# MarvelMathesh/sincformer-metacog-speech-enhancement

Measured on AMD Instinct MI355X. Metric: audio frames/sec/GPU (16 kHz, 512-frame utts) + mask RMSE vs CPU ref, higher is better.
Workload: dtype fp16 MFMA operands (PerceptionAgent, fusion, Conformer GEMMs, heads) + bf16 attention core, fp32 accumulate (ops.POLICIES['mixed']); 1 GPU; B256 x 512-frame utterances (L40880, T512) forward; batch_per_gpu=256, samples=40880, frames_per_utt=512, launch=eager launches, streams=2, precision_policy=mixed

## Files before the change

sincformer_metacog_speech_enhancement_amd/csrc/sinc_fir16.hip:

```cpp
#include "sfm_common.h"

#define FIR_C 64
#define FIR_KP 272
#define FIR_WROW 280
#define FIR_WAVES 8
#define FIR_SUB (FIR_WAVES * 256)
#define FIR_NSUB 4
#define FIR_XPT ((FIR_SUB + FIR_KP + FIR_WAVES * 64 - 1) / (FIR_WAVES * 64))
#define FIR_SPAN (FIR_SUB + FIR_KP)

template <class T>
__global__ __launch_bounds__(256) void sinc_fir16_prep_kernel(const float* __restrict__ filt, u16* __restrict__ wsh, int K) {
  const int o = blockIdx.x, c = blockIdx.y;
  for (int kp = threadIdx.x; kp < FIR_KP; kp += 256) {
    const int k = kp - o;
    const float h = (k >= 0 && k < K) ? filt[c * K + k] * 4096.0f : 0.f;
    const u16 hi = T::from_f32(h);
    const u16 lo = T::from_f32(h - T::to_f32(hi));
    wsh[(((long long)o * 2 + 0) * FIR_C + c) * FIR_KP + kp] = hi;
    wsh[(((long long)o * 2 + 1) * FIR_C + c) * FIR_KP + kp] = lo;
  }
}

template <class T, int PASSES>
__global__ __launch_bounds__(FIR_WAVES * 64) void sinc_fir16_kernel(const float* __restrict__ sig, const u16* __restrict__ wsh,
                                                         void* __restrict__ out, float* __restrict__ gn_partial,
                                                         int L, int pad, int out_f32, int tiles_per_batch) {
  extern __shared__ __attribute__((aligned(16))) unsigned char dsm[];
  u16* Wh = reinterpret_cast<u16*>(dsm);
  u16* Wl = Wh + FIR_C * FIR_WROW;
  u16* Xh = Wl + FIR_C * FIR_WROW;
  u16* Xl = Xh + FIR_SPAN;
  float* img = reinterpret_cast<float*>(Xl + FIR_SPAN);

  const int tid = threadIdx.x, lane = tid & 63, wave = tid >> 6;
  const int l31 = lane & 31, hl = lane >> 5;
  const int o = blockIdx.x, b = blockIdx.z;
  const int c0 = blockIdx.y * (FIR_NSUB * FIR_SUB);
  const float* xb = sig + (long long)b * L;

  {
    const u16* src = wsh + (long long)o * 2 * FIR_C * FIR_KP;
    for (int e = tid; e < 2 * FIR_C * (FIR_KP / 8); e += FIR_WAVES * 64) {
      const int part = e / (FIR_C * (FIR_KP / 8));
      const int rem = e - part * (FIR_C * (FIR_KP / 8));
      const int c = rem / (FIR_KP / 8), k8 = (rem - c * (FIR_KP / 8)) * 8;
      const u32x4 v = *reinterpret_cast<const u32x4*>(src + ((long long)part * FIR_C + c) * FIR_KP + k8);
      *reinterpret_cast<u32x4*>((part ? Wl : Wh) + c * FIR_WROW + k8) = v;
    }
  }

  constexpr int NT = FIR_WAVES * 64;
  float xr[FIR_XPT];
  auto load_span = [&](int m0) {
#pragma unroll
    for (int q = 0; q < FIR_XPT; ++q) {
      const int i = tid + q * NT;
      const int sidx = m0 + i - pad;
      xr[q] = (i < FIR_SPAN && sidx >= 0 && sidx < L) ? xb[sidx] : 0.f;
    }
  };
  load_span(c0);
  for (int sub = 0; sub < FIR_NSUB; ++sub) {
    const int m0 = c0 + sub * FIR_SUB;
    if (m0 >= L) break;
    __syncthreads();
#pragma unroll
    for (int q = 0; q < FIR_XPT; ++q) {
      const int i = tid + q * NT;
      if (i < FIR_SPAN) {
        const u16 hi = T::from_f32(xr[q]);
        Xh[i] = hi;
        Xl[i] = T::from_f32(xr[q] - T::to_f32(hi));
      }
    }
    __syncthreads();
    if (sub + 1 < FIR_NSUB && m0 + FIR_SUB < L) load_span(m0 + FIR_SUB);

    f32x16 acc[2];
#pragma unroll
    for (int j = 0; j < 2; ++j)
#pragma unroll
      for (int r = 0; r < 16; ++r) acc[j][r] = 0.f;
    const int xoff = wave * 256 + 8 * l31 + 8 * hl;
#pragma unroll
    for (int k0 = 0; k0 < FIR_KP; k0 += 16) {
      const u32x4 ah = *reinterpret_cast<const u32x4*>(Xh + xoff + k0);
      const u32x4 al = *reinterpret_cast<const u32x4*>(Xl + xoff + k0);
#pragma unroll
      for (int j = 0; j < 2; ++j) {
        const int wo = (j * 32 + l31) * FIR_WROW + k0 + 8 * hl;
        const u32x4 bh = *reinterpret_cast<const u32x4*>(Wh + wo);
        const u32x4 bl = *reinterpret_cast<const u32x4*>(Wl + wo);
        acc[j] = T::mfma(ah, bh, acc[j]);
        if (PASSES == 3) {
          acc[j] = T::mfma(ah, bl, acc[j]);
          acc[j] = T::mfma(al, bh, acc[j]);
        }
      }
    }

    float* im = img + wave * (32 * 68);
#pragma unroll
    for (int j = 0; j < 2; ++j)
#pragma unroll
      for (int r = 0; r < 16; ++r) im[mfma_row(r, lane) * 68 + j * 32 + l31] = acc[j][r] * (1.0f / 4096.0f);
    __builtin_amdgcn_s_waitcnt(0xC07F);
    __builtin_amdgcn_wave_barrier();
    const int c8 = (lane & 7) * 8, rsub = lane >> 3;
    float gsum = 0.f, gsq = 0.f;
#pragma unroll
    for (int r0 = 0; r0 < 32; r0 += 8) {
      const int row = r0 + rsub;
      const int m = m0 + wave * 256 + o + 8 * row;
      const f32x4 x0 = *reinterpret_cast<const f32x4*>(&im[row * 68 + c8]);
      const f32x4 x1 = *reinterpret_cast<const f32x4*>(&im[row * 68 + c8 + 4]);
      if (m < L) {
        const float v[8] = {x0[0], x0[1], x0[2], x0[3], x1[0], x1[1], x1[2], x1[3]};
#pragma unroll
        for (int e = 0; e < 8; ++e) { gsum += v[e]; gsq += v[e] * v[e]; }
        const long long off = ((long long)b * L + m) * FIR_C + c8;
        if (out_f32) {
          float* op = reinterpret_cast<float*>(out) + off;
          *reinterpret_cast<f32x4*>(op) = x0;
          *reinterpret_cast<f32x4*>(op + 4) = x1;
        } else {
          u32x4 pk;
#pragma unroll
          for (int e = 0; e < 4; ++e) pk[e] = pack2<T>(v[2 * e], v[2 * e + 1]);
          *reinterpret_cast<u32x4*>(reinterpret_cast<u16*>(out) + off) = pk;
        }
      }
    }
    if (gn_partial) {
      for (int s = 8; s < 64; s <<= 1) {
        gsum += __shfl_xor(gsum, s, 64);
        gsq += __shfl_xor(gsq, s, 64);
      }
      if (lane < 8) {
        const long long tile = ((long long)blockIdx.y * FIR_NSUB + sub) * (8 * FIR_WAVES) + o * FIR_WAVES + wave;
        const long long slot = (((long long)b * tiles_per_batch + tile) * 8 + lane) * 2;
        gn_partial[slot] = gsum;
        gn_partial[slot + 1] = gsq;
      }
    }
  }
}

extern "C" int sfm_sinc_fir16_tiles(int L) {
  const int chunk = FIR_NSUB * FIR_SUB;
  const int nchunks = (L + chunk - 1) / chunk;
  return nchunks * FIR_NSUB * 8 * FIR_WAVES;
}

template <class T, int PASSES>
static int sinc_fir16_go(const float* wave, const float* filt, void* wsh, void* out, float* gn_partial, int L, int K, int out_f32,
                         dim3 grid, int lds, int tpb, hipStream_t st) {
  SFM_LAUNCH((sinc_fir16_prep_kernel<T>), dim3(8, FIR_C), dim3(256), 0, st, filt, (u16*)wsh, K);
  SFM_LAUNCH_LDS((sinc_fir16_kernel<T, PASSES>), grid, dim3(FIR_WAVES * 64), lds, st, wave, (const u16*)wsh, out, gn_partial, L,
                 K / 2, out_f32, tpb);
  return SFM_OK;
}

extern "C" int sfm_sinc_fir16_ex(const float* wave, const float* filt, void* wsh, void* out, float* gn_partial, int B, int L, int C,
                                 int K, int out_f32, int dtype, int passes, void* stream) {
  if (!wave || !filt || !wsh || !out) return SFM_ERR_ARG;
  if (C != FIR_C || K < 1 || K + 7 > FIR_KP || (K & 1) == 0 || B <= 0 || L <= 0 || (passes != 0 && passes != 1 && passes != 3))
    return SFM_ERR_SHAPE;
  hipStream_t st = (hipStream_t)stream;
  const int chunk = FIR_NSUB * FIR_SUB;
  const int nchunks = (L + chunk - 1) / chunk;
  const int lds = (2 * FIR_C * FIR_WROW + 2 * FIR_SPAN) * 2 + FIR_WAVES * 32 * 68 * 4;
  const int tpb = nchunks * FIR_NSUB * 8 * FIR_WAVES;
  dim3 grid(8, nchunks, B);
  if (passes == 0) passes = (dtype == SFM_DT_F16 && out_f32 == 0) ? 1 : 3;
  if (dtype == SFM_DT_F16)
    return passes == 1 ? sinc_fir16_go<F16, 1>(wave, filt, wsh, out, gn_partial, L, K, out_f32, grid, lds, tpb, st)
                       : sinc_fir16_go<F16, 3>(wave, filt, wsh, out, gn_partial, L, K, out_f32, grid, lds, tpb, st);
  return passes == 1 ? sinc_fir16_go<BF16, 1>(wave, filt, wsh, out, gn_partial, L, K, out_f32, grid, lds, tpb, st)
                     : sinc_fir16_go<BF16, 3>(wave, filt, wsh, out, gn_partial, L, K, out_f32, grid, lds, tpb, st);
}

extern "C" int sfm_sinc_fir16(const float* wave, const float* filt, void* wsh, void* out, float* gn_partial, int B,
                              int L, int C, int K, int out_f32, int dtype, void* stream) {
  return sfm_sinc_fir16_ex(wave, filt, wsh, out, gn_partial, B, L, C, K, out_f32, dtype, 0, stream);
}
```

sincformer_metacog_speech_enhancement_amd/ops.py:

```python
import ctypes
import math
import numpy as np
import torch

from . import lib as _lib

EPI_NONE, EPI_SWISH, EPI_GELU, EPI_RESID, EPI_GLU, EPI_SIGMOID, EPI_TANH_SCALE, EPI_SIGMA, EPI_CPEA = range(9)

_DT_ID = {torch.bfloat16: 0, torch.float16: 1}
import os as _os
TRAIN_DTYPE = torch.float16
_state = {"dtype": TRAIN_DTYPE}

_SWITCHES = {
    "gemm_variant": ["SFM_GEMM_VARIANT", 0, 0],
    "attention_variant": [None, 0, 0],
    "lin256": ["SFM_LIN256", True, True],
    "headpool": ["SFM_HEADPOOL", True, True],
    "lstm_w16": ["SFM_LSTM_W16", True, True],
    "deterministic": ["SFM_DETERMINISTIC", True, True],
    "wgrad_stream": ["SFM_WGRAD_STREAM", True, True],
    "fuse_ffn_swish": ["SFM_FUSE_FFN_SWISH", True, True],
    "fuse_next_drop": ["SFM_FUSE_NEXT_DROP", True, True],
    "steal_grads": ["SFM_STEAL_GRADS", False, False],
# ... 528 lines not shown
        else:
            v = 2 if T >= 1024 else 1
    return {1: "attn_fwd_hd64_kernel", 2: "attn_fwd_hd64x2_kernel", 3: "attn_fwd_hd64r_kernel", 4: "attn_fwd_hd64p8_kernel",
            5: "attn_fwd_hd64p4_kernel", 6: "attn_fwd_hd64q4_kernel"}[v]


def set_attention_variant(v):
    v = int(v)
    if not 0 <= v <= 6:
        raise ValueError("attention variant %d" % v)
    _SWITCHES["attention_variant"][2] = v


def attention(qkv16, B, T, H, hd, out=None, prescaled=False, out_dtype=None):
    _need_dev(qkv16)
    L = _lib.load()
    D = H * hd
    ld = qkv16.stride(0)
    if qkv16.dtype != _state["dtype"]:
        raise RuntimeError("attention: Q | K | V are %s, the stage's format is %s" % (qkv16.dtype, _state["dtype"]))
    if out is None:
        out = torch.empty(B * T, D, device=qkv16.device, dtype=out_dtype or qkv16.dtype)
    _call("attention_fwd", L.sfm_attention_fwd_ex, (_p(qkv16), _p(out), B, T, H, hd, ld, out.stride(0), D, 2 * D, T * ld,
                                                    T * out.stride(0), (-1.0 if prescaled else 1.0 / math.sqrt(hd)), _dt(),
                                                    _DT_ID[out.dtype], switch("attention_variant"), _stream()),
          *_cost_of("attention_fwd", locals()))
    return out


LAYERNORM_MAX_D = 512


def layernorm(x32, w, b, out16=None, out32=None, act=0, eps=1e-5):
    _need_dev(x32)
    L = _lib.load()
    M, D = x32.shape[0], w.numel()
    if D > LAYERNORM_MAX_D:
        raise RuntimeError("layernorm: width %d is not supported (the LayerNorm kernels take D <= %d)" % (D, LAYERNORM_MAX_D))
    _call("layernorm", L.sfm_layernorm, (_p(x32), _p(w), _p(b), _p(out16), _p(out32), M, D, x32.stride(0),
                         out16.stride(0) if out16 is not None else 0, out32.stride(0) if out32 is not None else 0,
                         eps, act, _dt(), _stream()),
          *_cost_of("layernorm", locals()))


def gn_finalize(partial, w, b, Bn, P, G, C, rows, eps=1e-5):
    L = _lib.load()
    scale = torch.empty(Bn, C, device=w.device, dtype=torch.float32)
    shift = torch.empty(Bn, C, device=w.device, dtype=torch.float32)
    _call("gn_finalize", L.sfm_gn_finalize, (_p(partial), _p(w), _p(b), _p(scale), _p(shift), Bn, P, G, C, rows, eps, _stream()),
          *_cost_of("gn_finalize", locals()))
    return scale, shift


def gn_apply(x1, sc1, sh1, out, Bn, rows, C, act=0, x2=None, sc2=None, sh2=None):
    L = _lib.load()
    in_f32 = 1 if x1.dtype == torch.float32 else 0
    out_f32 = 1 if out.dtype == torch.float32 else 0
    _call("gn_apply", L.sfm_gn_apply, (_p(x1), _p(sc1), _p(sh1), _p(x2), _p(sc2), _p(sh2), _p(out), Bn, rows, C, in_f32, out_f32, act,
                        _dt(), _stream()),
          *_cost_of("gn_apply", locals()))
    return out


def dwconv_bn_swish(x16, wdw, bdw, bnw, bnb, bnm, bnv, B, T, C, out=None, eps=1e-5):
    L = _lib.load()
    KS = wdw.shape[-1]
    if out is None:
        out = torch.empty_like(x16)
    _call("dwconv_bn_swish", L.sfm_dwconv_bn_swish, (_p(x16), _p(wdw), _p(bdw), _p(bnw), _p(bnb), _p(bnm), _p(bnv), _p(out), B, T, C, KS,
                               eps, _dt(), _stream()),
          *_cost_of("dwconv_bn_swish", locals()))
    return out


def dwconv_folded(x16, wT, sc, sh, B, T, C, out=None, act=1):
    L = _lib.load()
    KS = wT.shape[0]
    if out is None:
        out = torch.empty_like(x16)
    _call("dwconv_bn_swish", L.sfm_dwconv_folded, (_p(x16), _p(wT), _p(sc), _p(sh), _p(out), B, T, C, KS, int(act),
                                                   1 if out.dtype == torch.float32 else 0, _dt(), _stream()),
          2.0 * B * T * C * KS, B * T * C * 4.0)
    return out


def convert_rows(src32, dst16, M, C, Cz, ld_src, ld_dst):
    L = _lib.load()
    _call("convert_rows", L.sfm_convert_rows, (_p(src32), _p(dst16), M, C, Cz, ld_src, ld_dst, _dt(), _stream()),
          *_cost_of("convert_rows", locals()), tag="M%d C%d" % (M, C))


def transpose(src, dst, B, R, C, src_batch, src_row, dst_batch, dst_row):
    L = _lib.load()
    _call("transpose", L.sfm_transpose, (_p(src), _p(dst), B, R, C, src_batch, src_row, dst_batch, dst_row,
                         1 if src.dtype == torch.float32 else 0, 1 if dst.dtype == torch.float32 else 0, _dt(),
                         _stream()),
          *_cost_of("transpose", locals()))


def mean_time(src32, B, T, C, ld_src):
    L = _lib.load()
    out = torch.empty(B, C, device=src32.device, dtype=torch.float32)
    scratch = torch.empty(int(L.sfm_mean_time_scratch_floats(B, T, C)), device=src32.device, dtype=torch.float32)
    _call("pool_time", L.sfm_mean_time, (_p(src32), _p(out), _p(scratch), B, T, C, ld_src, _stream()), 0.0, 4.0 * B * T * C)
    return out


def pool_time_bwd(dout32, B, Tin, Tout, C):
    L = _lib.load()
    dout32 = dout32.contiguous()
    dsrc = torch.empty(B, Tin, C, device=dout32.device, dtype=torch.float32)
    _call("pool_time_bwd", L.sfm_pool_time_bwd, (_p(dout32), _p(dsrc), B, Tin, Tout, C, C, C, _stream()), 0.0,
          4.0 * B * (Tin + Tout) * C)
    return dsrc


def pool_time(src32, dst16, dst32, B, Tin, Tout, C, ld_src, ld_dst, scale=None, shift=None):
    L = _lib.load()
    src_bytes = src32.element_size()
    if src_bytes == 4:
        args = (_p(src32), _p(scale), _p(shift), _p(dst16), _p(dst32), B, Tin, Tout, C, ld_src, ld_dst, _dt(), _stream())
        fn = L.sfm_pool_time_affine
    else:
        args = (_p(src32), _DT_ID[src32.dtype], _p(scale), _p(shift), _p(dst16), _p(dst32), B, Tin, Tout, C, ld_src, ld_dst,
                _dt(), _stream())
        fn = L.sfm_pool_time_affine16
    _call("pool_time", fn, args, *_cost_of("pool_time", locals()))


def stft_lognorm_pack(re, im, dst16, M, F, zpad, ld_dst):
    L = _lib.load()
    _call("stft_lognorm_pack", L.sfm_stft_lognorm_pack, (_p(re), _p(im), _p(dst16), M, F, zpad, ld_dst, _dt(), _stream()),
          *_cost_of("stft_lognorm_pack", locals()))


def polar_mask(lm, lp, B, rows, F, phase_scale, ld_logits, mag_bias=None, nr=None, ni=None, mr=None, mi=None, er=None,
               ei=None, mmag=None, ld_enh=0):
    L = _lib.load()
    _call("polar_mask", L.sfm_polar_mask, (_p(lm), _p(lp), _p(mag_bias), _p(nr), _p(ni), _p(mr), _p(mi), _p(er), _p(ei), _p(mmag), B,
                          rows, F, float(phase_scale), ld_logits, ld_enh, _stream()),
          *_cost_of("polar_mask", locals()))


def complex_mul(sr, si, mr, mi):
    L = _lib.load()
    er, ei = torch.empty_like(sr), torch.empty_like(sr)
    _call("complex_mul", L.sfm_complex_mul, (_p(sr), _p(si), _p(mr), _p(mi), _p(er), _p(ei), sr.numel(), _stream()),
          *_cost_of("complex_mul", locals()))
    return er, ei


def istft_ola(frames, win2, out, B, T, Ln, n_fft, hop, win, ld_frames):
    L = _lib.load()
    _call("istft_ola", L.sfm_istft_ola, (_p(frames), _p(win2), _p(out), B, T, Ln, n_fft, hop, win, ld_frames, _stream()),
          *_cost_of("istft_ola", locals()))


ATTN_QTILE = 128
DWCONV_TILE = 64
_XCDS, _XCD_RUN = 8, 8


def attention_items(frame_counts, H):
    T = np.asarray(frame_counts, dtype=np.int64)
    order = np.argsort(-T, kind="stable")
    nt = (T[order] + ATTN_QTILE - 1) // ATTN_QTILE
    per = np.repeat(nt, H)
    n = int(per.sum())
    utt = np.repeat(np.repeat(order, H), per)
    head = np.repeat(np.tile(np.arange(H), len(T)), per)
    first = np.repeat(np.cumsum(per) - per, per)
    tile = np.arange(n) - first
    logical = np.stack([utt, head, tile, np.zeros(n, dtype=np.int64)], axis=1)
    run = _XCDS * _XCD_RUN
    pos = np.arange(n)
    base = pos // run * run
    total = np.minimum(run, n - base)
    p = pos - base
    q, r, xcd, slot = total // _XCDS, total % _XCDS, p % _XCDS, p // _XCDS
    src = base + np.where(xcd < r, xcd * (q + 1), r * (q + 1) + (xcd - r) * q) + slot
    return np.ascontiguousarray(logical[src], dtype=np.int32)


def dwconv_tiles(frame_counts):
    T = np.asarray(frame_counts, dtype=np.int64)
    nt = (T + DWCONV_TILE - 1) // DWCONV_TILE
    n = int(nt.sum())
    utt = np.repeat(np.arange(len(T)), nt)
    tile = np.arange(n) - np.repeat(np.cumsum(nt) - nt, nt)
    return np.ascontiguousarray(np.stack([utt, tile], axis=1), dtype=np.int32)


def framed_gemm_varlen(sig, Wt, out, samp_off, frame_off, *, B, sum_T, hop, padl, K, N, ldm, ldn=1, mode=0, out2=None, nsplit=0):
    _need_dev(sig, Wt, out, samp_off, frame_off)
    L = _lib.load()
    Kpad, Npad = Wt.shape
    _call("framed_gemm_f32_varlen", L.sfm_framed_gemm_f32_varlen,
          (_p(sig), _p(Wt), _p(out), _p(out2), _p(samp_off), _p(frame_off), B, sum_T, hop, padl, K, Kpad, N, Npad, nsplit, ldm, ldn,
           mode, 1 if out.dtype == torch.float32 else 0, _dt(), _stream()),
          2.0 * sum_T * N * K, 4.0 * (sig.numel() + sum_T * N))
    return out


def framed_gemm_split16_varlen(sig, W, out, samp_off, frame_off, *, B, sum_T, hop, padl, ldm, mode=0, out2=None, nsplit=0,
                               col2_off=0):
    _need_dev(sig, out, samp_off, frame_off)
    L = _lib.load()
    hi, lo, K, N = W
    Npad, Kpad = hi.shape
    _call("framed_gemm_split16_varlen", L.sfm_framed_gemm_split16_varlen,
          (_p(sig), _p(hi), _p(lo), _p(out), _p(out2), _p(samp_off), _p(frame_off), B, sum_T, hop, padl, K, Kpad, N, Npad, nsplit,
           col2_off, ldm, mode, _stream()),
          2.0 * sum_T * K * N, 4.0 * (sig.numel() + sum_T * N))
    return out


def attention_varlen(qkv16, frame_off, items, B, max_T, sum_T, H, hd, out=None, prescaled=False, out_dtype=None, sum_T2=None):
    _need_dev(qkv16, frame_off, items)
    L = _lib.load()
    D = H * hd
    ld = qkv16.stride(0)
    if qkv16.dtype != _state["dtype"]:
        raise RuntimeError("attention: Q | K | V are %s, the stage's format is %s" % (qkv16.dtype, _state["dtype"]))
    if out is None:
        out = torch.empty(sum_T, D, device=qkv16.device, dtype=out_dtype or qkv16.dtype)
    n_items = 0 if items is None else items.shape[0]
    _call("attention_fwd_varlen", L.sfm_attention_fwd_varlen,
          (_p(qkv16), _p(out), _p(frame_off), _p(items), n_items, B, max_T, sum_T, H, hd, ld, out.stride(0), D, 2 * D,
           (-1.0 if prescaled else 1.0 / math.sqrt(hd)), _dt(), _DT_ID[out.dtype], _stream()),
          4.0 * H * hd * float(sum_T2 if sum_T2 is not None else 0), 4.0 * sum_T * D * 2)
    return out


def dwconv_folded_varlen(x16, wT, sc, sh, frame_off, tiles, B, max_T, sum_T, C, out=None, act=1):
    _need_dev(x16, frame_off, tiles)
    L = _lib.load()
    KS = wT.shape[0]
    if out is None:
        out = torch.empty_like(x16)
    _call("dwconv_varlen", L.sfm_dwconv_folded_varlen,
          (_p(x16), _p(wT), _p(sc), _p(sh), _p(out), _p(frame_off), _p(tiles), 0 if tiles is None else tiles.shape[0], B, max_T,
           sum_T, C, KS, int(act), 1 if out.dtype == torch.float32 else 0, _dt(), _stream()),
          2.0 * sum_T * C * KS, sum_T * C * 4.0)
    return out


def istft_ola_varlen(frames, win2, out, frame_off, samp_off, B, n_fft, hop, win, ld_frames):
    _need_dev(frames, out, frame_off, samp_off)
    L = _lib.load()
    _call("istft_ola_varlen", L.sfm_istft_ola_varlen,
          (_p(frames), _p(win2), _p(out), _p(frame_off), _p(samp_off), B, out.numel(), n_fft, hop, win, ld_frames, _stream()),
          0.0, out.numel() * 12.0)
    return out


def pack_spec(re, im, dst, M, F, ld, ld_src):
    L = _lib.load()
    _call("pack_spec", L.sfm_pack_spec, (_p(re), _p(im), _p(dst), M, F, ld, ld_src, _stream()),
          *_cost_of("pack_spec", locals()))


def sinc_filters(low_hz, band_hz, window, n_, C, K, sample_rate, min_low_hz, min_band_hz, want_filt=True):
    L = _lib.load()
    dev = low_hz.device
    Npad = round_up(C, 64)
    Wt = torch.zeros(round_up(K, 32), Npad, device=dev, dtype=torch.float32)
    filt = torch.empty(C, K, device=dev, dtype=torch.float32) if want_filt else None
    _call("sinc_filters", L.sfm_sinc_filters, (_p(low_hz), _p(band_hz), _p(window), _p(n_), _p(filt), _p(Wt), C, K, Npad,
                            float(sample_rate), float(min_low_hz), float(min_band_hz), _stream()),
          *_cost_of("sinc_filters", locals()))
    return filt, Wt


def ffn_fused(x32, lnw, lnb, w1_16, b1, w2_16, b2, alpha=0.5, eps=1e-5, out=None):
    _need_dev(x32)
    Lb = _lib.load()
    M, D = x32.shape
    FF = w1_16.shape[0]
    if out is None:
        out = torch.empty_like(x32)
    _call("ffn_fused", Lb.sfm_ffn_fused, (_p(x32), _p(lnw), _p(lnb), _p(w1_16), _p(b1), _p(w2_16), _p(b2), _p(out), M, D, FF,
                                          float(alpha), float(eps), _dt(), _stream()), 4.0 * M * D * FF, M * D * 8.0)
    return out


def ffn_fused_ln(x32, lnw, lnb, w1_16, b1, w2_16, b2, ln2w, ln2b, ln_f32, want_y=True, alpha=0.5, eps=1e-5):
    _need_dev(x32)
    Lb = _lib.load()
    M, D = x32.shape
    FF = w1_16.shape[0]
    y = torch.empty_like(x32) if want_y else None
    ln = torch.empty(M, D, device=x32.device, dtype=torch.float32 if ln_f32 else _state["dtype"])
    _call("ffn_fused", Lb.sfm_ffn_fused_ln, (_p(x32), _p(lnw), _p(lnb), _p(w1_16), _p(b1), _p(w2_16), _p(b2), _p(y), M, D, FF,
                                             float(alpha), float(eps), _p(ln2w), _p(ln2b), _p(ln), 1 if ln_f32 else 0, _dt(),
                                             _stream()), 4.0 * M * D * FF, M * D * (8.0 if want_y else 4.0) + M * D * (4.0 if ln_f32 else 2.0))
    return y, ln


def sinc_fir16(wave, filt, out, B, L, C, K, want_stats=True, passes=0):
    Lb = _lib.load()
    dev = wave.device
    wsh = torch.empty(8 * 2 * 64 * 272, device=dev, dtype=torch.int16)
    P = Lb.sfm_sinc_fir16_tiles(L)
    part = torch.zeros(B, P, 8, 2, device=dev, dtype=torch.float32) if want_stats else None
    out_f32 = 1 if out.dtype == torch.float32 else 0
    flops, nbytes = 2.0 * B * L * C * K, B * L * 4 + B * L * C * (4 if out_f32 else 2)
    _call("sinc_fir16", Lb.sfm_sinc_fir16_ex, (_p(wave), _p(filt), _p(wsh), _p(out), _p(part), B, L, C, K, out_f32, _dt(), int(passes),
                                               _stream()), flops, nbytes)
    return part, P


def wave_moments(est, tgt):
    L = _lib.load()
    B, Ln = est.shape
    S = torch.zeros(B, 5, device=est.device, dtype=torch.float64)
    _call("loss_reduce", L.sfm_wave_moments, (_p(est), _p(tgt), _p(S), B, Ln, _p(_ws(64 * B * 5, est.device, torch.float64)), _stream()),
          0.0, 8.0 * B * Ln)
    return S


def wave_moments_varlen(est, tgt, samp_off, B, max_L):
    _need_dev(est, tgt, samp_off)
    L = _lib.load()
    S = torch.zeros(B, 5, device=est.device, dtype=torch.float64)
    _call("loss_reduce", L.sfm_wave_moments_varlen, (_p(est), _p(tgt), _p(S), _p(samp_off), B, int(max_L), _stream()), 0.0,
          8.0 * est.numel())
    return S


def ssnr_frames_varlen(clean, enh, samp_off, frame_off, B, sum_frames, frame, hop, upper=35.0, lower=-10.0):
    _need_dev(clean, enh, samp_off, frame_off)
    L = _lib.load()
    acc = torch.zeros(B, 2, device=clean.device, dtype=torch.float64)
    _call("metrics", L.sfm_ssnr_frames_varlen, (_p(clean), _p(enh), _p(acc), _p(samp_off), _p(frame_off), B, int(sum_frames),
                                                int(frame), int(hop), float(upper), float(lower), _stream()), 0.0,
          8.0 * clean.numel() * frame / hop)
    return acc


def stoi_frames_varlen(cr, ci, er, ei, sc, se, frame_off, B):
    _need_dev(cr, ci, er, ei, sc, se, frame_off)
    L = _lib.load()
    n, F = cr.shape
    acc = torch.zeros(B, device=cr.device, dtype=torch.float64)
    _call("metrics", L.sfm_stoi_frames_varlen, (_p(cr), _p(ci), _p(er), _p(ei), _p(sc), _p(se), _p(acc), _p(frame_off), B, n, F,
                                                _stream()), 0.0, 16.0 * n * F)
    return acc


def lsd_frames(cr, ci, er, ei):
    _need_dev(cr, ci, er, ei)
    L = _lib.load()
    B, n, F = cr.shape
    acc = torch.zeros(B, device=cr.device, dtype=torch.float64)
    _call("metrics", L.sfm_lsd_frames, (_p(cr), _p(ci), _p(er), _p(ei), _p(acc), B, n, F, _stream()), 0.0, 16.0 * B * n * F)
    return acc


def lsd_frames_varlen(cr, ci, er, ei, frame_off, B):
    _need_dev(cr, ci, er, ei, frame_off)
    L = _lib.load()
    n, F = cr.shape
    acc = torch.zeros(B, device=cr.device, dtype=torch.float64)
    _call("metrics", L.sfm_lsd_frames_varlen, (_p(cr), _p(ci), _p(er), _p(ei), _p(acc), _p(frame_off), B, n, F, _stream()), 0.0,
          16.0 * n * F)
    return acc


def _ws64(n, device):
    t = _ws(n, device, torch.float64)
    return t if t is not None else torch.empty(int(n), device=device, dtype=torch.float64)


def pstoi_loss(enh, clean, band_w, need_grad=False, frame_len=30, beta=15.0):
    pair = isinstance(enh, (tuple, list))
    e0, e1 = enh if pair else (enh, None)
    c0, c1 = clean if pair else (clean, None)
    _need_dev(e0, e1, c0, c1, band_w)
    L = _lib.load()
    if pair:
        B, T, F = e0.shape
    else:
        B, F, T = e0.shape
    NB = band_w.shape[0]
    FL = int(frame_len)
    if band_w.shape[1] != F or c0.shape != e0.shape or NB > 32 or F > 257 or not 2 <= FL <= 32 or T < FL:
        _lib.check(-2, "pstoi_loss")
    loss = torch.empty(1, device=e0.device, dtype=torch.float32)
    g0 = torch.empty_like(e0) if need_grad else None
    g1 = torch.empty_like(e0) if need_grad and pair else None
    S = T // FL
    n = e0.numel()
    _call("pstoi_loss", L.sfm_pstoi_loss, (_p(e0), _p(e1), _p(c0), _p(c1), _p(band_w), _p(loss), _p(g0), _p(g1),
                                           _p(_ws64(B * S + 1, e0.device)), B, T, F, NB, FL, float(beta), 1 if pair else 0,
                                           _stream()),
          (6.0 if need_grad else 4.0) * NB * F * B * S * FL,
          pstoi_bytes(B, T, F, FL, pair, need_grad))
    return loss, ((g0, g1) if pair else g0) if need_grad else None


def pstoi_bytes(B, T, F, frame_len, pair, need_grad):
    used, every = 4.0 * B * (T // frame_len) * frame_len * F, 4.0 * B * T * F
    if pair:
        return 4 * used + ((2 * used + 2 * every) if need_grad else 0.0)
    return 2 * used + (every if need_grad else 0.0)


def mse_loss(pred, target, need_grad=False):
    _need_dev(pred, target)
    L = _lib.load()
    if pred.shape != target.shape or pred.numel() == 0:
        _lib.check(-2, "mse_loss")
    loss = torch.empty(1, device=pred.device, dtype=torch.float32)
    grad = torch.empty_like(pred) if need_grad else None
    n = pred.numel()
    _call("mse_loss", L.sfm_mse_loss, (_p(pred), _p(target), _p(loss), _p(grad), _p(_ws64(1025, pred.device)), n, _stream()),
          3.0 * n, (12.0 if need_grad else 8.0) * n)
    return loss, grad


def spec_sums(pr, pi, tr, ti, out=None):
    L = _lib.load()
    S = torch.zeros(4, device=pr.device, dtype=torch.float64) if out is None else out
    _call("loss_reduce", L.sfm_spec_sums, (_p(pr), _p(pi), _p(tr), _p(ti), _p(S), pr.numel(),
                                           _p(_ws(2048 * 4, pr.device, torch.float64)), _stream()), 0.0, 16.0 * pr.numel())
    return S


def enhancer_loss_finalize(Sw, Sm, Sr, nr, B, Ln, n_mag, R=None):
    L = _lib.load()
    out = torch.empty(4, device=Sw.device, dtype=torch.float32)
    _call("loss_reduce", L.sfm_enhancer_loss_finalize, (_p(Sw), _p(Sm), _p(Sr), _p(nr), B, Ln, n_mag,
                                                        Sr.shape[0] if R is None else int(R), _p(out), _stream()))
    return out


def sisnr_bwd(est, tgt, Sw, dwave, scale=1.0):
    L = _lib.load()
    B, Ln = est.shape
    _call("loss_bwd", L.sfm_sisnr_bwd, (_p(est), _p(tgt), _p(Sw), _p(dwave), B, Ln, float(scale), _stream()), 0.0, 12.0 * B * Ln)


def spec_loss_bwd(pr, pi, tr, ti, S, dr, di, F, ld, mode, accumulate=False, scale=1.0):
    L = _lib.load()
    _call("loss_bwd", L.sfm_spec_loss_bwd, (_p(pr), _p(pi), _p(tr), _p(ti), _p(S), _p(dr), _p(di), pr.numel(), F, ld, mode,
                                            1 if accumulate else 0, float(scale), _stream()), 0.0, 24.0 * pr.numel())


def stft_adjoint_ola(frames, dwave, B, T, Ln, n_fft, hop, win, accumulate=True, post=None):
    L = _lib.load()
    _call("loss_bwd", L.sfm_stft_adjoint_ola, (_p(frames), _p(dwave), _p(post), B, T, Ln, n_fft, hop, win,
                                               1 if accumulate else 0, _stream()), 0.0, 4.0 * (B * T * win + 2 * B * Ln))


def polar_mask_bwd(lm, lp, nr, ni, der, dei, dlog, M, F, phase_scale, ld_logits, mag_bias=None, rows_per_batch=None):
    L = _lib.load()
    _call("loss_bwd", L.sfm_polar_mask_bwd, (_p(lm), _p(lp), _p(mag_bias), _p(nr), _p(ni), _p(der), _p(dei), _p(dlog), M,
                                             rows_per_batch or M, F, float(phase_scale), ld_logits, dlog.stride(0), _stream()),
          0.0, 32.0 * M * F)


def sum_time(src32, B, T, C, ld_src):
    L = _lib.load()
    out = torch.empty(B, C, device=src32.device, dtype=torch.float32)
    scratch = torch.empty(int(L.sfm_mean_time_scratch_floats(B, T, C)), device=src32.device, dtype=torch.float32)
    _call("pool_time", L.sfm_sum_time, (_p(src32), _p(out), _p(scratch), B, T, C, ld_src, _stream()), 0.0, 4.0 * B * T * C)
    return out


def _tn_ws(L_, M, N, K, device):
    if not switch("deterministic"):
        return None, 0
    n = int(L_.sfm_tn_ws_floats(M, N, K))
    return _ws(n, device), n


def sinc_wgrad(wave, dy, C, K, exact=False):
    L_ = _lib.load()
    B, L = wave.shape
    if not exact and K == 251 and dy.dtype == _state["dtype"] and C % 8 == 0:
        Lc = int(L_.sfm_sinc_shift_len(L))
        xs = torch.empty(B, 8, Lc, device=wave.device, dtype=dy.dtype)
        _call("sinc_shift_pack", L_.sfm_sinc_shift_pack, (_p(wave), _p(xs), B, L, _dt(), _stream()), 0.0, B * (4.0 * L + 16.0 * Lc))
        dW = torch.zeros(C, 256, device=wave.device, dtype=torch.float32)
        ws, wsn = _tn_ws(L_, B * L, C, 256, wave.device)
        _call("sinc_wgrad16", L_.sfm_sinc_wgrad16, (_p(dy), _p(xs), _p(dW), B, L, C, _dt(), _p(ws), wsn, _stream()),
              2.0 * B * L * C * 256, B * L * (2.0 * C + 16.0))
        return dW[:, :K].contiguous()
    dfilt = torch.zeros(C, K, device=wave.device, dtype=torch.float32)
    scratch = torch.empty(int(L_.sfm_sinc_wgrad_scratch_floats(B, L, C, K)), device=wave.device, dtype=torch.float32)
    _call("sinc_wgrad", L_.sfm_sinc_wgrad, (_p(wave), _p(dy), 1 if dy.dtype == torch.float32 else 0, _p(dfilt), _p(scratch), B, L, C,
                                            K, _dt(), _stream()), 2.0 * B * L * C * K, B * L * (4.0 + C * dy.element_size()))
    return dfilt


def gn_stats(partial, rows, C, G):
    s = partial.double().sum(dim=1)
    n = float(rows * (C // G))
    mean = s[..., 0] / n
    var = (s[..., 1] / n - mean * mean).clamp_min(0.0)
    return mean.float(), torch.rsqrt(var + 1e-5).float()


def gn_act_backward(dout, act, G, x1, sc1, sh1, mean1, rstd1, gamma1, x2=None, sc2=None, sh2=None, mean2=None, rstd2=None,
                    gamma2=None, dx_dtype=None):
    L_ = _lib.load()
    B, L, C = x1.shape
    dx_dtype = dx_dtype or _state["dtype"]
    two = x2 is not None
    dev = x1.device
    f32 = lambda t: 1 if t.dtype == torch.float32 else 0
    c32 = lambda t: None if t is None else t.float().contiguous()
    dout = dout.contiguous()
    sc1, sh1, mean1, rstd1, gamma1 = c32(sc1), c32(sh1), c32(mean1), c32(rstd1), c32(gamma1)
    sc2, sh2, mean2, rstd2, gamma2 = c32(sc2), c32(sh2), c32(mean2), c32(rstd2), c32(gamma2)
    work = torch.zeros(3 * B * C + 3 * C, device=dev, dtype=torch.float32)
    S, dparam = work[:3 * B * C], work[3 * B * C:].view(3, C)
    nbytes = float(B * L * C) * ((4 if f32(dout) else 2) + (1 + two) * (4 if f32(x1) else 2))
    ws = _ws(int(L_.sfm_gn_bwd_reduce_ws_floats(B, L, C)), dev) if switch("deterministic") else None
    _call("gn_bwd_reduce", L_.sfm_gn_bwd_reduce, (_p(dout), f32(dout), _p(x1), f32(x1), _p(sc1), _p(sh1), _p(mean1), _p(rstd1), _p(x2),
                                           f32(x2) if two else 0, _p(sc2), _p(sh2), _p(mean2), _p(rstd2), _p(S), B, L, C, G,
                                           int(act), _dt(), _p(ws), _stream()), 0.0, nbytes)
    coef = torch.empty(2, 3, B, C, device=dev, dtype=torch.float32)
    _call("gn_bwd_coefs", L_.sfm_gn_bwd_coefs, (_p(S), _p(gamma1), _p(rstd1), _p(gamma2), _p(rstd2), _p(coef[0]),
                                                _p(coef[1]) if two else None, _p(dparam), B, L, C, G, _stream()), 0.0,
          4.0 * 9 * B * C)
    dx1 = torch.empty(B, L, C, device=dev, dtype=dx_dtype)
    dx2 = torch.empty(B, L, C, device=dev, dtype=dx_dtype) if two else None
    _call("gn_bwd_apply", L_.sfm_gn_bwd_apply, (_p(dout), f32(dout), _p(x1), f32(x1), _p(sc1), _p(sh1), _p(mean1), _p(rstd1), _p(coef[0]),
                                          _p(dx1), f32(dx1), _p(x2), f32(x2) if two else 0, _p(sc2), _p(sh2), _p(mean2), _p(rstd2),
                                          _p(coef[1]) if two else None, _p(dx2), f32(dx2) if two else 0, B, L, C, G, int(act),
                                          _dt(), _stream()), 0.0, nbytes + float(B * L * C) * (1 + two) * (4 if f32(dx1) else 2))
    if two:
        return dx1, dparam[1], dparam[0], dx2, dparam[2], dparam[0]
    return dx1, dparam[1], dparam[0]


_WGRAD = {"stream": None, "keep": []}


class wgrad_side_stream:

    def __init__(self, enabled=True):
        self.enabled = enabled and switch("wgrad_stream")

    def __enter__(self):
        if self.enabled:
            if "side" not in _WGRAD:
                _WGRAD["side"] = torch.cuda.Stream()
            _WGRAD["stream"] = _WGRAD["side"]
        return self

    def __exit__(self, *exc):
        if self.enabled:
            torch.cuda.current_stream().wait_stream(_WGRAD["side"])
            _WGRAD["stream"] = None
            _WGRAD["keep"].clear()
        return False


class after_wgrad:

    def __init__(self, *temporaries):
        self.ws = _WGRAD["stream"]
        self.tmp = temporaries
        self.ctx = None

    def __enter__(self):
        if self.ws is not None:
            self.ctx = torch.cuda.stream(self.ws)
            self.ctx.__enter__()
        return self

    def __exit__(self, *exc):
        if self.ws is not None:
            self.ctx.__exit__(*exc)
            _WGRAD["keep"].extend(self.tmp)
        return False


def gemm16_tn(G16, X16, dW, db=None):
    ws = _WGRAD["stream"]
    if ws is not None and torch.cuda.current_stream() != ws:
        ws.wait_stream(torch.cuda.current_stream())
        with torch.cuda.stream(ws):
            gemm16_tn(G16, X16, dW, db)
        _WGRAD["keep"].extend((G16, X16))
        return
    L = _lib.load()
    M, N = G16.shape
    K = X16.shape[1]
    ws, wsn = _tn_ws(L, M, N, K, G16.device)
    _call("gemm16_tn", L.sfm_gemm16_tn, (_p(G16), _p(X16), _p(dW), _p(db), M, N, K, G16.stride(0), X16.stride(0), dW.stride(0),
                                         _dt(), _p(ws), wsn, _stream()), 2.0 * M * N * K, M * (N + K) * 2.0,
          tag="M%d N%d K%d" % (M, N, K))


def conv_wgrad16(dy16, x16, B, Lout, Lin, Cin, N, ksize, stride, pad):
    ws = _WGRAD["stream"]
    if ws is not None and torch.cuda.current_stream() != ws:
        ws.wait_stream(torch.cuda.current_stream())
        with torch.cuda.stream(ws):
            out = conv_wgrad16(dy16, x16, B, Lout, Lin, Cin, N, ksize, stride, pad)
        _WGRAD["keep"].extend((dy16, x16))
        return out
    L = _lib.load()
    buf = torch.zeros(N * ksize * Cin + N, device=x16.device, dtype=torch.float32)
# ... 350 lines not shown
```

Baseline: 8.617 million STFT frames/s (whole job).

## Add register-resident-weight single-pass sinc FIR kernel with run-based grid and compact stats

Adds a new single-pass sinc FIR kernel that keeps filter weights in registers instead of LDS. It uses 4-wave blocks with two blocks per CU, double-buffered input spans loaded through buffer loads, and a software-pipelined MFMA loop. Outputs are staged through LDS so global stores are coalesced, and the grid is sized to the CU count with runs of sub-tiles per block. GroupNorm partial stats are reduced per block into a compact layout, so the zero-fill of the partial buffer is dropped. The three-pass split kernel is kept for higher precision and adapted to the new stats layout. The cost is much higher register pressure and a changed stats layout that downstream consumers must match.

```diff
diff --git a/sincformer_metacog_speech_enhancement_amd/csrc/sinc_fir16.hip b/sincformer_metacog_speech_enhancement_amd/csrc/sinc_fir16.hip
--- a/sincformer_metacog_speech_enhancement_amd/csrc/sinc_fir16.hip
+++ b/sincformer_metacog_speech_enhancement_amd/csrc/sinc_fir16.hip
@@ -8,6 +8,11 @@
 #define FIR_NSUB 4
 #define FIR_XPT ((FIR_SUB + FIR_KP + FIR_WAVES * 64 - 1) / (FIR_WAVES * 64))
 #define FIR_SPAN (FIR_SUB + FIR_KP)
+#define FIRR_WAVES 4
+#define FIRR_SUB (FIRR_WAVES * 256)
+#define FIRR_SPAN (FIRR_SUB + FIR_KP)
+#define FIRR_XPT ((FIRR_SPAN + FIRR_WAVES * 64 - 1) / (FIRR_WAVES * 64))
+#define FIRR_KS (FIR_KP / 16)
 
 template <class T>
 __global__ __launch_bounds__(256) void sinc_fir16_prep_kernel(const float* __restrict__ filt, u16* __restrict__ wsh, int K) {
@@ -22,16 +27,17 @@
   }
 }
 
-template <class T, int PASSES>
+template <class T>
 __global__ __launch_bounds__(FIR_WAVES * 64) void sinc_fir16_kernel(const float* __restrict__ sig, const u16* __restrict__ wsh,
                                                          void* __restrict__ out, float* __restrict__ gn_partial,
-                                                         int L, int pad, int out_f32, int tiles_per_batch) {
+                                                         int L, int pad, int out_f32, int ntile) {
   extern __shared__ __attribute__((aligned(16))) unsigned char dsm[];
   u16* Wh = reinterpret_cast<u16*>(dsm);
   u16* Wl = Wh + FIR_C * FIR_WROW;
   u16* Xh = Wl + FIR_C * FIR_WROW;
   u16* Xl = Xh + FIR_SPAN;
   float* img = reinterpret_cast<float*>(Xl + FIR_SPAN);
+  float* red = img + FIR_WAVES * 32 * 68;
 
   const int tid = threadIdx.x, lane = tid & 63, wave = tid >> 6;
   const int l31 = lane & 31, hl = lane >> 5;
@@ -60,11 +66,25 @@
       xr[q] = (i < FIR_SPAN && sidx >= 0 && sidx < L) ? xb[sidx] : 0.f;
     }
   };
+  auto fold_partials = [&](int m0) {
+    if (gn_partial && tid < 32) {
+      const int half = tid >> 4, v = tid & 15;
+      const int tile = m0 / FIRR_SUB + half;
+      if (tile < ntile) {
+        const float* r = red + half * 4 * 16 + v;
+        const float tot = ((r[0] + r[16]) + r[32]) + r[48];
+        gn_partial[((((long long)b * ntile + tile) * 8 + o) * 8 + (v >> 1)) * 2 + (v & 1)] = tot;
+      }
+    }
+  };
   load_span(c0);
+  int mprev = -1;
   for (int sub = 0; sub < FIR_NSUB; ++sub) {
     const int m0 = c0 + sub * FIR_SUB;
     if (m0 >= L) break;
     __syncthreads();
+    if (mprev >= 0) fold_partials(mprev);
+    mprev = m0;
 #pragma unroll
     for (int q = 0; q < FIR_XPT; ++q) {
       const int i = tid + q * NT;
@@ -93,10 +113,8 @@
         const u32x4 bh = *reinterpret_cast<const u32x4*>(Wh + wo);
         const u32x4 bl = *reinterpret_cast<const u32x4*>(Wl + wo);
         acc[j] = T::mfma(ah, bh, acc[j]);
-        if (PASSES == 3) {
-          acc[j] = T::mfma(ah, bl, acc[j]);
-          acc[j] = T::mfma(al, bh, acc[j]);
-        }
+        acc[j] = T::mfma(ah, bl, acc[j]);
+        acc[j] = T::mfma(al, bh, acc[j]);
       }
     }
 
@@ -138,47 +156,224 @@
         gsq += __shfl_xor(gsq, s, 64);
       }
       if (lane < 8) {
-        const long long tile = ((long long)blockIdx.y * FIR_NSUB + sub) * (8 * FIR_WAVES) + o * FIR_WAVES + wave;
-        const long long slot = (((long long)b * tiles_per_batch + tile) * 8 + lane) * 2;
-        gn_partial[slot] = gsum;
-        gn_partial[slot + 1] = gsq;
-      }
-    }
-  }
+        red[wave * 16 + lane * 2] = gsum;
+        red[wave * 16 + lane * 2 + 1] = gsq;
+      }
+    }
+  }
+  __syncthreads();
+  if (mprev >= 0) fold_partials(mprev);
+}
+
+template <class T, bool OUT32>
+__global__ __launch_bounds__(FIRR_WAVES * 64, 2) void sinc_fir16r_kernel(const float* __restrict__ sig, const u16* __restrict__ wsh,
+                                                                         void* __restrict__ out, float* __restrict__ gn_partial,
+                                                                         int L, int pad, int nsub, int run_len) {
+  constexpr int ROWB = OUT32 ? 272 : 144;
+  constexpr int NT = FIRR_WAVES * 64;
+  __shared__ __attribute__((aligned(16))) u16 X[2][FIRR_SPAN];
+  __shared__ __attribute__((aligned(16))) unsigned char img[FIRR_WAVES][32 * ROWB];
+  __shared__ float red[2][FIRR_WAVES][16];
+
+  const int tid = threadIdx.x, lane = tid & 63, wave = tid >> 6;
+  const int l31 = lane & 31, hl = lane >> 5;
+  const int o = blockIdx.x, b = blockIdx.z;
+  const int s0 = blockIdx.y * run_len, s1 = min(s0 + run_len, nsub);
+  if (s0 >= s1) return;
+  const float* xb = sig + (long long)b * L;
+
+  u32x4 wt[2][FIRR_KS];
+  {
+    const u16* wp = wsh + ((long long)o * 2 * FIR_C + l31) * FIR_KP + 8 * hl;
+#pragma unroll
+    for (int j = 0; j < 2; ++j)
+#pragma unroll
+      for (int ks = 0; ks < FIRR_KS; ++ks) wt[j][ks] = *reinterpret_cast<const u32x4*>(wp + j * 32 * FIR_KP + ks * 16);
+  }
+
+  float xr[FIRR_XPT];
+  auto xrs = __builtin_amdgcn_make_buffer_rsrc((void*)xb, 0, L * 4, 0x00020000);
+  auto load_span = [&](int m0) {
+#pragma unroll
+    for (int q = 0; q < FIRR_XPT; ++q) {
+      const int sidx = m0 + tid + q * NT - pad;
+      xr[q] = __builtin_bit_cast(float, __builtin_amdgcn_raw_buffer_load_b32(xrs, sidx * 4, 0, 0));
+    }
+  };
+  auto store_span = [&](u16* Xd) {
+#pragma unroll
+    for (int q = 0; q < FIRR_XPT; ++q) {
+      const int i = tid + q * NT;
+      if (i < FIRR_SPAN) Xd[i] = T::from_f32(xr[q]);
+    }
+  };
+  auto write_partial = [&](int sub, const float* r) {
+    const int v = tid;
+    const float tot = ((r[v] + r[16 + v]) + r[32 + v]) + r[48 + v];
+    gn_partial[((((long long)b * nsub + sub) * 8 + o) * 8 + (v & 7)) * 2 + (v >> 3)] = tot;
+  };
+
+  load_span(s0 * FIRR_SUB);
+  store_span(X[0]);
+  __builtin_amdgcn_s_waitcnt(0x0F70);
+  int cur = 0;
+  for (int s = s0; s < s1; ++s, cur ^= 1) {
+    const int m0 = s * FIRR_SUB;
+    __syncthreads();
+    if (gn_partial && s > s0 && tid < 16) write_partial(s - 1, &red[cur ^ 1][0][0]);
+    const bool more = s + 1 < s1;
+    if (more) load_span(m0 + FIRR_SUB);
+
+    f32x16 acc[2];
+#pragma unroll
+    for (int j = 0; j < 2; ++j)
+#pragma unroll
+      for (int r = 0; r < 16; ++r) acc[j][r] = 0.f;
+    const u16* xp = X[cur] + wave * 256 + 8 * l31 + 8 * hl;
+    u32x4 xv[4];
+#pragma unroll
+    for (int ks = 0; ks < 3; ++ks) xv[ks] = *reinterpret_cast<const u32x4*>(xp + ks * 16);
+    __builtin_amdgcn_sched_group_barrier(0x100, 3, 0);
+#pragma unroll
+    for (int ks = 0; ks < FIRR_KS; ++ks) {
+      if (ks + 3 < FIRR_KS) {
+        xv[(ks + 3) & 3] = *reinterpret_cast<const u32x4*>(xp + (ks + 3) * 16);
+        __builtin_amdgcn_sched_group_barrier(0x100, 1, 0);
+      }
+#pragma unroll
+      for (int j = 0; j < 2; ++j) acc[j] = T::mfma(wt[j][ks], xv[ks & 3], acc[j]);
+      __builtin_amdgcn_sched_group_barrier(0x008, 2, 0);
+    }
+    if (more) store_span(X[cur ^ 1]);
+
+    const int mbase = m0 + wave * 256 + o;
+    const bool rowok = mbase + 8 * l31 < L;
+    float v16[16];
+#pragma unroll
+    for (int j = 0; j < 2; ++j)
+#pragma unroll
+      for (int gq = 0; gq < 4; ++gq) {
+        float s_ = 0.f, q_ = 0.f;
+#pragma unroll
+        for (int e = 0; e < 4; ++e) {
+          const float v = acc[j][4 * gq + e] * (1.0f / 4096.0f);
+          acc[j][4 * gq + e] = v;
+          if (rowok) {
+            s_ += v;
+            q_ = __builtin_fmaf(v, v, q_);
+          }
+        }
+        v16[j * 4 + gq] = s_;
+        v16[8 + j * 4 + gq] = q_;
+      }
+    if (gn_partial) {
+      const float tot = wave_sum16_transpose(v16, lane);
+      if (lane < 16) red[cur][wave][lane] = tot;
+    }
+    unsigned char* im = img[wave];
+    __builtin_amdgcn_s_waitcnt(0xC07F);
+    __builtin_amdgcn_wave_barrier();
+    if (!OUT32) {
+#pragma unroll
+      for (int j = 0; j < 2; ++j)
+#pragma unroll
+        for (int gq = 0; gq < 4; ++gq) {
+          u32x2 w;
+          w[0] = pack2<T>(acc[j][4 * gq + 0], acc[j][4 * gq + 1]);
+          w[1] = pack2<T>(acc[j][4 * gq + 2], acc[j][4 * gq + 3]);
+          *reinterpret_cast<u32x2*>(im + l31 * ROWB + (j * 32 + 8 * gq + 4 * hl) * 2) = w;
+        }
+      __builtin_amdgcn_s_waitcnt(0xC07F);
+      __builtin_amdgcn_wave_barrier();
+      u32x4 rv[4];
+#pragma unroll
+      for (int k = 0; k < 4; ++k) {
+        const int c = lane + 64 * k;
+        rv[k] = *reinterpret_cast<const u32x4*>(im + (c >> 3) * ROWB + (c & 7) * 16);
+      }
+#pragma unroll
+      for (int k = 0; k < 4; ++k) {
+        const int c = lane + 64 * k;
+        const int m = mbase + 8 * (c >> 3);
+        if (m < L) *reinterpret_cast<u32x4*>(reinterpret_cast<u16*>(out) + ((long long)b * L + m) * FIR_C + (c & 7) * 8) = rv[k];
+      }
+    } else {
+#pragma unroll
+      for (int j = 0; j < 2; ++j)
+#pragma unroll
+        for (int gq = 0; gq < 4; ++gq)
+          *reinterpret_cast<f32x4*>(im + l31 * ROWB + (j * 32 + 8 * gq + 4 * hl) * 4) =
+              f32x4{acc[j][4 * gq + 0], acc[j][4 * gq + 1], acc[j][4 * gq + 2], acc[j][4 * gq + 3]};
+      __builtin_amdgcn_s_waitcnt(0xC07F);
+      __builtin_amdgcn_wave_barrier();
+      u32x4 rv[8];
+#pragma unroll
+      for (int k = 0; k < 8; ++k) {
+        const int c = lane + 64 * k;
+        rv[k] = *reinterpret_cast<const u32x4*>(im + (c >> 4) * ROWB + (c & 15) * 16);
+      }
+#pragma unroll
+      for (int k = 0; k < 8; ++k) {
+        const int c = lane + 64 * k;
+        const int m = mbase + 8 * (c >> 4);
+        if (m < L) *reinterpret_cast<u32x4*>(reinterpret_cast<float*>(out) + ((long long)b * L + m) * FIR_C + (c & 15) * 4) = rv[k];
+      }
+    }
+  }
+  __syncthreads();
+  if (gn_partial && tid < 16) write_partial(s1 - 1, &red[cur ^ 1][0][0]);
 }
 
 extern "C" int sfm_sinc_fir16_tiles(int L) {
+  return ((L + FIRR_SUB - 1) / FIRR_SUB) * 8;
+}
+
+template <class T>
+static int sinc_fir16_one_pass(const float* wave, const float* filt, void* wsh, void* out, float* gn_partial, int B, int L, int K,
+                               int out_f32, hipStream_t st) {
+  const int ntile = (L + FIRR_SUB - 1) / FIRR_SUB;
+  SFM_LAUNCH((sinc_fir16_prep_kernel<T>), dim3(8, FIR_C), dim3(256), 0, st, filt, (u16*)wsh, K);
+  const int ncu = sfm_cu_count();
+  if (ncu <= 0) return SFM_ERR_LAUNCH;
+  const long long want = (8LL * ncu + 8LL * B - 1) / (8LL * B);
+  const int nruns0 = (int)(want < 1 ? 1 : want > ntile ? ntile : want);
+  const int run_len = (ntile + nruns0 - 1) / nruns0;
+  const int nruns = (ntile + run_len - 1) / run_len;
+  dim3 grid(8, nruns, B);
+  if (out_f32)
+    SFM_LAUNCH((sinc_fir16r_kernel<T, true>), grid, dim3(FIRR_WAVES * 64), 0, st, wave, (const u16*)wsh, out, gn_partial, L, K / 2,
+               ntile, run_len);
+  else
+    SFM_LAUNCH((sinc_fir16r_kernel<T, false>), grid, dim3(FIRR_WAVES * 64), 0, st, wave, (const u16*)wsh, out, gn_partial, L, K / 2,
+               ntile, run_len);
+  return SFM_OK;
+}
+
+template <class T>
+static int sinc_fir16_split(const float* wave, const float* filt, void* wsh, void* out, float* gn_partial, int B, int L, int K,
+                            int out_f32, hipStream_t st) {
+  const int ntile = (L + FIRR_SUB - 1) / FIRR_SUB;
+  SFM_LAUNCH((sinc_fir16_prep_kernel<T>), dim3(8, FIR_C), dim3(256), 0, st, filt, (u16*)wsh, K);
   const int chunk = FIR_NSUB * FIR_SUB;
-  const int nchunks = (L + chunk - 1) / chunk;
-  return nchunks * FIR_NSUB * 8 * FIR_WAVES;
-}
-
-template <class T, int PASSES>
-static int sinc_fir16_go(const float* wave, const float* filt, void* wsh, void* out, float* gn_partial, int L, int K, int out_f32,
-                         dim3 grid, int lds, int tpb, hipStream_t st) {
-  SFM_LAUNCH((sinc_fir16_prep_kernel<T>), dim3(8, FIR_C), dim3(256), 0, st, filt, (u16*)wsh, K);
-  SFM_LAUNCH_LDS((sinc_fir16_kernel<T, PASSES>), grid, dim3(FIR_WAVES * 64), lds, st, wave, (const u16*)wsh, out, gn_partial, L,
-                 K / 2, out_f32, tpb);
+  const int lds = (2 * FIR_C * FIR_WROW + 2 * FIR_SPAN) * 2 + FIR_WAVES * 32 * 68 * 4 + FIR_WAVES * 16 * 4;
+  dim3 grid(8, (L + chunk - 1) / chunk, B);
+  SFM_LAUNCH_LDS((sinc_fir16_kernel<T>), grid, dim3(FIR_WAVES * 64), lds, st, wave, (const u16*)wsh, out, gn_partial, L, K / 2,
+                 out_f32, ntile);
   return SFM_OK;
 }
 
 extern "C" int sfm_sinc_fir16_ex(const float* wave, const float* filt, void* wsh, void* out, float* gn_partial, int B, int L, int C,
                                  int K, int out_f32, int dtype, int passes, void* stream) {
   if (!wave || !filt || !wsh || !out) return SFM_ERR_ARG;
-  if (C != FIR_C || K < 1 || K + 7 > FIR_KP || (K & 1) == 0 || B <= 0 || L <= 0 || (passes != 0 && passes != 1 && passes != 3))
+  if (C != FIR_C || K < 1 || K + 7 > FIR_KP || (K & 1) == 0 || B <= 0 || L <= 0 || L >= (1 << 29) || (passes != 0 && passes != 1 && passes != 3))
     return SFM_ERR_SHAPE;
   hipStream_t st = (hipStream_t)stream;
-  const int chunk = FIR_NSUB * FIR_SUB;
-  const int nchunks = (L + chunk - 1) / chunk;
-  const int lds = (2 * FIR_C * FIR_WROW + 2 * FIR_SPAN) * 2 + FIR_WAVES * 32 * 68 * 4;
-  const int tpb = nchunks * FIR_NSUB * 8 * FIR_WAVES;
-  dim3 grid(8, nchunks, B);
   if (passes == 0) passes = (dtype == SFM_DT_F16 && out_f32 == 0) ? 1 : 3;
   if (dtype == SFM_DT_F16)
-    return passes == 1 ? sinc_fir16_go<F16, 1>(wave, filt, wsh, out, gn_partial, L, K, out_f32, grid, lds, tpb, st)
-                       : sinc_fir16_go<F16, 3>(wave, filt, wsh, out, gn_partial, L, K, out_f32, grid, lds, tpb, st);
-  return passes == 1 ? sinc_fir16_go<BF16, 1>(wave, filt, wsh, out, gn_partial, L, K, out_f32, grid, lds, tpb, st)
-                     : sinc_fir16_go<BF16, 3>(wave, filt, wsh, out, gn_partial, L, K, out_f32, grid, lds, tpb, st);
+    return passes == 1 ? sinc_fir16_one_pass<F16>(wave, filt, wsh, out, gn_partial, B, L, K, out_f32, st)
+                       : sinc_fir16_split<F16>(wave, filt, wsh, out, gn_partial, B, L, K, out_f32, st);
+  return passes == 1 ? sinc_fir16_one_pass<BF16>(wave, filt, wsh, out, gn_partial, B, L, K, out_f32, st)
+                     : sinc_fir16_split<BF16>(wave, filt, wsh, out, gn_partial, B, L, K, out_f32, st);
 }
 
 extern "C" int sfm_sinc_fir16(const float* wave, const float* filt, void* wsh, void* out, float* gn_partial, int B,
diff --git a/sincformer_metacog_speech_enhancement_amd/ops.py b/sincformer_metacog_speech_enhancement_amd/ops.py
--- a/sincformer_metacog_speech_enhancement_amd/ops.py
+++ b/sincformer_metacog_speech_enhancement_amd/ops.py
@@ -854,7 +854,7 @@
     dev = wave.device
     wsh = torch.empty(8 * 2 * 64 * 272, device=dev, dtype=torch.int16)
     P = Lb.sfm_sinc_fir16_tiles(L)
-    part = torch.zeros(B, P, 8, 2, device=dev, dtype=torch.float32) if want_stats else None
+    part = torch.empty(B, P, 8, 2, device=dev, dtype=torch.float32) if want_stats else None
     out_f32 = 1 if out.dtype == torch.float32 else 0
     flops, nbytes = 2.0 * B * L * C * K, B * L * 4 + B * L * C * (4 if out_f32 else 2)
     _call("sinc_fir16", Lb.sfm_sinc_fir16_ex, (_p(wave), _p(filt), _p(wsh), _p(out), _p(part), B, L, C, K, out_f32, _dt(), int(passes),
```

New measurement: 8.753 million STFT frames/s (whole job) (median of 6 runs). 1.6% higher.
